# EspressoSystems/Push-CDN

Hardware: NVIDIA H100
Metric: broadcast fan-out egress GB/s (1 KiB x 2^20 subscribers per GPU, 1 topic); msgs/s and % of HBM peak alongside (higher is better)
Workload: dtype u8

## Files before the change

push-cdn_b200/csrc/kernels.cu:

```cuda
#include "kernels.cuh"

#include <atomic>

#include "frame_parse_core.h"

namespace pcdn {

std::atomic<unsigned long long> g_kernel_launches{0};
#define PCDN_COUNT_LAUNCH (void)g_kernel_launches.fetch_add(1, std::memory_order_relaxed)

unsigned long long kernel_launches() { return g_kernel_launches.load(std::memory_order_relaxed); }
void count_kernel_launch() { PCDN_COUNT_LAUNCH; }

__device__ __forceinline__ uint32_t lane_id() { return threadIdx.x & 31; }

__device__ __forceinline__ uint32_t warp_incl_scan(uint32_t v) {
  const uint32_t lane = lane_id();
#pragma unroll
  for (int o = 1; o < 32; o <<= 1) {
    uint32_t n = __shfl_up_sync(0xffffffffu, v, o);
    if (lane >= (uint32_t)o) v += n;
  }
  return v;
}
// ... 354 lines not shown
  const uint32_t p4 = p3 + __popc(hi.x), p5 = p4 + __popc(hi.y), p6 = p5 + __popc(hi.z), p7 = p6 + __popc(hi.w);
  const uint32_t incl = warp_incl_scan(p7), ex = incl - p7;
  uint32_t last = 0;
  if (lane == 31) {
    w.cnt[(size_t)j * s.nblk + blk] = incl;
    __threadfence();
    last = atomicAdd(&w.done[j], 1u) == s.nblk - 1 ? 1u : 0u;
  }
  uint4* Bo = reinterpret_cast<uint4*>(w.B + (size_t)j * s.W + w0);
  Bo[0] = lo; Bo[1] = hi;
  uint4 pre;
  pre.x = ex | ((ex + p0) << 16); pre.y = (ex + p1) | ((ex + p2) << 16);
  pre.z = (ex + p3) | ((ex + p4) << 16); pre.w = (ex + p5) | ((ex + p6) << 16);
  *reinterpret_cast<uint4*>(w.wpre + (size_t)j * s.W + w0) = pre;
  if (__shfl_sync(0xffffffffu, last, 31)) {
    __threadfence();
    uint32_t carry = 0;
    for (uint32_t bb = 0; bb < s.nblk; bb += 32) {
      const uint32_t i = bb + lane;
      const uint32_t v = i < s.nblk ? __ldcg(w.cnt + (size_t)j * s.nblk + i) : 0;
      const uint32_t in = warp_incl_scan(v);
      if (i < s.nblk) w.base[(size_t)j * s.nblk + i] = carry + in - v;
      carry += __shfl_sync(0xffffffffu, in, 31);
    }
    if (lane == 0) { w.D[m] = carry; w.jidx[m] = j; w.done[j] = 0; }
  }
}
void launch_match(const DevState& s, const Work& w, const BatchIn& b, cudaStream_t st) {
  if (!b.n_bcast) return;
  dim3 grid((s.nblk + 7) / 8, b.n_bcast);
  PCDN_COUNT_LAUNCH, k_match<<<grid, 256, 0, st>>>(s, b, w);
}

__device__ __forceinline__ uint32_t frame_vec_bytes(uint32_t raw_len) { return (4u + raw_len + 15u) & ~15u; }
__device__ __forceinline__ uint32_t frame_units(uint32_t raw_len) { return (4u + raw_len + kUnit - 1u) / kUnit; }
__device__ __forceinline__ uint32_t rec_units(const DevState& s, uint32_t raw_len) {
  return s.shared_payload ? 1u : frame_units(raw_len);
}
__device__ __forceinline__ uint32_t tile_recipients(uint32_t frame_bytes, uint32_t tile_bytes) {
  const uint32_t chunk = min(frame_bytes, kChunkBytes);
  return max(32u, min(kTileRecipients, tile_bytes / chunk));
}

__device__ __forceinline__ void plan_classify(const DevState& s, const BatchIn& b, uint32_t m, uint32_t d, uint32_t* cls_out,
                                              uint32_t* tiles_out) {
  uint32_t cls = CLS_THIN, tiles = 0;
  if (d >= kFatMin) {
    const uint32_t len = b.raw_len[m];
    const bool dense = s.cm_enable && ((uint64_t)d << kCmDenseShift) >= s.N && b.kind[m] == 4;
    if (dense && frame_units(len) * kUnit <= kCmMaxBytes) {
      cls = CLS_CM;
    } else {
      cls = CLS_FAT;
      const uint32_t nch = (frame_vec_bytes(len) + kChunkBytes - 1) / kChunkBytes;
      const uint32_t tr = tile_recipients(frame_vec_bytes(len), s.fat_tile_bytes);
      tiles = nch * ((d + tr - 1) / tr);
    }
  }
  *cls_out = cls; *tiles_out = tiles;
}

__global__ void __launch_bounds__(256) k_plan_a(DevState s, BatchIn b, Work w, uint32_t nblk) {
  __shared__ uint32_t sm[9];
  const uint32_t m = blockIdx.x * 256 + threadIdx.x;
  const bool valid = m < b.n_msgs;
  const uint32_t d = valid ? w.D[m] : 0;
  uint32_t cls, tiles;
  plan_classify(s, b, m, d, &cls, &tiles);
  uint32_t tot;
  uint32_t e0 = block256_excl_scan(cls != CLS_THIN ? d : 0, &tot, sm);
  if (threadIdx.x == 0) w.scan_tmp[blockIdx.x] = tot;
  uint32_t e1 = block256_excl_scan(cls == CLS_THIN ? d : 0, &tot, sm);
  if (threadIdx.x == 0) w.scan_tmp[nblk + blockIdx.x] = tot;
  uint32_t e2 = block256_excl_scan(tiles, &tot, sm);
  if (threadIdx.x == 0) w.scan_tmp[2 * nblk + blockIdx.x] = tot;
  uint32_t e3 = block256_excl_scan(cls == CLS_CM ? 1u : 0u, &tot, sm);
  if (threadIdx.x == 0) w.scan_tmp[3 * nblk + blockIdx.x] = tot;
  if (valid) { w.eb_fat[m] = e0; w.eb_thin[m] = e1; w.tbase[m] = e2; w.cm_rank[m] = e3; w.cls[m] = (uint8_t)cls; }
  if (gridDim.x == 1) {
    if (valid && cls == CLS_CM) w.cm_list[e3] = m;
    if (threadIdx.x == 0) {
      const uint32_t t0 = w.scan_tmp[0], t1 = w.scan_tmp[1], t2 = w.scan_tmp[2], t3 = w.scan_tmp[3];
      w.stats->n_fat_entries = t0; w.stats->n_thin_entries = t1; w.stats->n_fat_tiles = t2; w.stats->tile_cursor = 0;
      w.stats->n_cm = t3; w.stats->cm_cursor = 0;
      if (t0 > w.cap_fat || t1 > w.cap_thin) w.stats->status = 1;
      const uint32_t n = b.n_msgs;
      w.eb_fat[n] = t0; w.eb_thin[n] = t1; w.tbase[n] = t2; w.cm_rank[n] = t3;
    }
  }
}
__global__ void __launch_bounds__(256) k_plan_b(Work w, uint32_t nblk) {
  __shared__ uint32_t sm[9];
  const uint32_t q = blockIdx.x;
  uint32_t* t = w.scan_tmp + (size_t)q * nblk;
  uint32_t carry = 0;
  for (uint32_t bb = 0; bb < nblk; bb += 256) {
    const uint32_t i = bb + threadIdx.x;
    const uint32_t v = i < nblk ? t[i] : 0;
    uint32_t tot, ex = block256_excl_scan(v, &tot, sm);
    if (i < nblk) t[i] = ex + carry;
    carry += tot;
  }
  if (threadIdx.x == 0) {
    if (q == 0) { w.stats->n_fat_entries = carry; if (carry > w.cap_fat) w.stats->status = 1; }
    if (q == 1) { w.stats->n_thin_entries = carry; if (carry > w.cap_thin) w.stats->status = 1; }
    if (q == 2) { w.stats->n_fat_tiles = carry; w.stats->tile_cursor = 0; }
    if (q == 3) { w.stats->n_cm = carry; w.stats->cm_cursor = 0; }
  }
}
__global__ void __launch_bounds__(256) k_plan_c(BatchIn b, Work w, uint32_t nblk) {
  const uint32_t m = blockIdx.x * 256 + threadIdx.x;
  if (m < b.n_msgs) {
    w.eb_fat[m] += w.scan_tmp[blockIdx.x];
    w.eb_thin[m] += w.scan_tmp[nblk + blockIdx.x];
    w.tbase[m] += w.scan_tmp[2 * nblk + blockIdx.x];
    const uint32_t r = w.cm_rank[m] + w.scan_tmp[3 * nblk + blockIdx.x];
    w.cm_rank[m] = r;
    if (w.cls[m] == CLS_CM) w.cm_list[r] = m;
  } else if (m == b.n_msgs) {
    w.eb_fat[m] = w.stats->n_fat_entries;
    w.eb_thin[m] = w.stats->n_thin_entries;
    w.tbase[m] = w.stats->n_fat_tiles;
    w.cm_rank[m] = w.stats->n_cm;
  }
}
void launch_plan(const DevState& s, const Work& w, const BatchIn& b, cudaStream_t st) {
  if (b.n_bcast == 0) return;
  const uint32_t nblk = (b.n_msgs + 255) / 256;
  PCDN_COUNT_LAUNCH, k_plan_a<<<nblk, 256, 0, st>>>(s, b, w, nblk);
  if (nblk == 1) return;
  PCDN_COUNT_LAUNCH, k_plan_b<<<4, 256, 0, st>>>(w, nblk);
  PCDN_COUNT_LAUNCH, k_plan_c<<<(b.n_msgs + 1 + 255) / 256, 256, 0, st>>>(b, w, nblk);
}

struct ConnCursor {
  uint32_t pt, us, bu;
  uint32_t s1_off, s1_units, s1_rec, s2_units, s2_rec;
  uint32_t ovf, in2;
  uint32_t bytes;
};
__device__ __forceinline__ uint32_t alloc_record(ConnCursor& k, uint32_t u, uint32_t R, uint32_t raw_len) {
  if (k.ovf) return kOffInvalid;
  const bool wrap = k.pt + u > R;
  const uint32_t pad = wrap ? R - k.pt : 0, at = wrap ? 0 : k.pt;
  if (u > R || k.us + pad + u > R) { k.ovf = 1; return kOffInvalid; }
  k.us += pad + u;
  k.bu += pad + u;
  if (wrap && k.s1_rec) k.in2 = 1;
  if (!k.in2) { if (!k.s1_rec) k.s1_off = at; k.s1_units += u; k.s1_rec++; }
  else { k.s2_units += u; k.s2_rec++; }
  k.pt = at + u;
  k.bytes += 4u + raw_len;
  return at;
}

__device__ __forceinline__ uint32_t pool_lookback(const Work& w, uint32_t vb, uint32_t ctot) {
  const uint32_t lane = lane_id();
  volatile unsigned long long* st = w.lb_state;
  const unsigned long long tag = (unsigned long long)w.stamp << 34;
  auto pack = [&](uint32_t flag, uint32_t v) { return tag | ((unsigned long long)flag << 32) | v; };
  unsigned long long prefix64 = 0;
  if (vb > 0) {
    if (lane == 0) st[vb] = pack(1u, ctot);
    int j = (int)vb - 1;
    for (;;) {
      const int idx = j - (int)lane;
      unsigned long long x = 0;
      if (idx >= 0) { do { x = st[idx]; } while ((x >> 34) != (tag >> 34)); }
      const uint32_t flag = idx >= 0 ? (uint32_t)(x >> 32) & 3u : 2u;
      const uint32_t val = idx >= 0 ? (uint32_t)x : 0u;
      const uint32_t pm = __ballot_sync(0xffffffffu, flag == 2u);
      const int first = pm ? __ffs(pm) - 1 : 32;
      const uint32_t v = (int)lane <= first ? val : 0u;
      const unsigned long long take = ((unsigned long long)__reduce_add_sync(0xffffffffu, v >> 16) << 16) + __reduce_add_sync(0xffffffffu, v & 0xFFFFu);
      prefix64 += take;
      if (pm) break;
      j -= 32;
    }
  }
  const uint32_t prefix = (uint32_t)(prefix64 > 0xFFFFFFFFull ? 0xFFFFFFFFull : prefix64);
  const unsigned long long incl = prefix64 + ctot;
  if (lane == 0) { __threadfence(); st[vb] = pack(2u, incl > 0xFFFFFFFFull ? 0xFFFFFFFFu : (uint32_t)incl); }
  return prefix;
}
__device__ __forceinline__ void pool_allocate(const DevState& s, const Work& w, unsigned long long total64) {
  PoolState* p = s.pool_state;
  BatchStats* bs = w.stats;
  if (w.pool_unblock) p->blocked = 0;
  if (total64 > s.pool_units) { bs->status = 3; return; }
  const uint32_t total = (uint32_t)total64;
// ... 220 lines not shown
__global__ void __cluster_dims__(8, 1, 1) __launch_bounds__(1024, 1)
k_ctrl_small(DevState s, BatchIn b, Work w, int zero_stats, BatchStats* publish, int offsets_only) {
  __shared__ uint32_t sm[33];
  __shared__ uint32_t gbase[5];
  const uint32_t tid = threadIdx.x, rank = blockIdx.x;
  if (zero_stats && rank == 0 && tid < sizeof(BatchStats) / 4) reinterpret_cast<uint32_t*>(w.stats)[tid] = 0;

  if (HAS_DIRECT && rank == 0 && !offsets_only) {
    __shared__ uint32_t skey_s[kSmallCtrlMsgs], sorted_s[kSmallCtrlMsgs];
    __syncthreads();
    for (uint32_t g0 = 0; g0 < b.n_msgs * 8; g0 += 1024) direct_lookup_body<false>(s, b, w, g0 + tid);
    __syncthreads();
    const uint32_t n = b.n_msgs;
    if (tid < n) { const uint32_t t = w.dconn[tid]; skey_s[tid] = t == kConnNone ? s.N : t; }
    __syncthreads();
    if (tid < n) {
      const uint32_t key = skey_s[tid];
      uint32_t r = 0;
      for (uint32_t o = 0; o < n; o++) r += (skey_s[o] < key || (skey_s[o] == key && o < tid)) ? 1u : 0u;
      sorted_s[r] = key;
      w.dlist[r] = tid;
    }
    __syncthreads();
    if (tid < n) {
      const uint32_t key = sorted_s[tid];
      if (tid == 0 || sorted_s[tid - 1] != key) { w.dstart[key] = tid; w.dstamp[key] = w.stamp; }
      if (tid + 1 == n || sorted_s[tid + 1] != key) w.dend[key] = tid + 1;
    }
  }

  if (!offsets_only) {
    const uint32_t q = tid >> 8, wl = tid & 255u, nitems = b.n_bcast * s.nblk;
    for (uint32_t i0 = rank * 4; i0 < nitems; i0 += 32) {
      const uint32_t it = i0 + q;
      const bool live = it < nitems;
      const uint32_t j = live ? it / s.nblk : 0, blk = live ? it % s.nblk : 0;
      const uint32_t wd = blk * kBlockWords + wl;
      const uint32_t word = live ? match_word(s, b, b.bcast_index[j], wd) : 0;
      uint32_t tot, ex = cta_excl_scan<32>(__popc(word), &tot, sm);
      if (wl == 0) gbase[q] = ex;
      if (tid == 0) gbase[4] = tot;
      __syncthreads();
      if (live) {
        w.B[(size_t)j * s.W + wd] = word;
        w.wpre[(size_t)j * s.W + wd] = (uint16_t)(ex - gbase[q]);
        if (wl == 0) w.cnt[(size_t)j * s.nblk + blk] = gbase[q + 1] - gbase[q];
      }
      __syncthreads();
    }
  }
  cluster_sync_all();

  if (rank == 0 && !offsets_only) {
    if (tid < b.n_bcast) {
      uint32_t carry = 0;
      for (uint32_t blk = 0; blk < s.nblk; blk++) {
        const uint32_t v = w.cnt[(size_t)tid * s.nblk + blk];
        w.base[(size_t)tid * s.nblk + blk] = carry;
        carry += v;
      }
      const uint32_t m = b.bcast_index[tid];
      w.D[m] = carry; w.jidx[m] = tid;
    }
    __syncthreads();
  }

  if (rank == 0 && !offsets_only) {
    const uint32_t m = tid;
    const bool valid = m < b.n_msgs;
    const uint32_t d = valid ? w.D[m] : 0;
    uint32_t cls, tiles;
    plan_classify(s, b, m, d, &cls, &tiles);
    uint32_t t0, t1, t2, t3;
    const uint32_t e0 = cta_excl_scan<32>(cls != CLS_THIN ? d : 0, &t0, sm);
    const uint32_t e1 = cta_excl_scan<32>(cls == CLS_THIN ? d : 0, &t1, sm);
    const uint32_t e2 = cta_excl_scan<32>(tiles, &t2, sm);
    const uint32_t e3 = cta_excl_scan<32>(cls == CLS_CM ? 1u : 0u, &t3, sm);
    if (valid) {
      w.eb_fat[m] = e0; w.eb_thin[m] = e1; w.tbase[m] = e2; w.cm_rank[m] = e3; w.cls[m] = (uint8_t)cls;
      if (cls == CLS_CM) w.cm_list[e3] = m;
    }
    if (tid == 0) {
      w.stats->n_fat_entries = t0; w.stats->n_thin_entries = t1; w.stats->n_fat_tiles = t2; w.stats->tile_cursor = 0;
      w.stats->n_cm = t3; w.stats->cm_cursor = 0;
      if (t0 > w.cap_fat || t1 > w.cap_thin) w.stats->status = 1;
      const uint32_t n = b.n_msgs;
      w.eb_fat[n] = t0; w.eb_thin[n] = t1; w.tbase[n] = t2; w.cm_rank[n] = t3;
    }
  }
  cluster_sync_all();

  for (uint32_t c0 = 0; c0 < s.N; c0 += 8192)
    offsets_body<HAS_DIRECT, 1024, true, true>(s, b, w, s.N, c0 + rank * 1024 + tid, c0 / 1024 + rank, s.N / 1024);

  if (publish) {
    cluster_sync_all();
    if (rank == 0 && tid < sizeof(BatchStats) / 4)
      reinterpret_cast<uint32_t*>(publish)[tid] = __ldcg(reinterpret_cast<const uint32_t*>(w.stats) + tid);
  }
}
void launch_ctrl_small(const DevState& s, const Work& w, const BatchIn& b, bool has_direct, bool zero_stats,
                       BatchStats* publish, bool offsets_only, cudaStream_t st) {
  if (has_direct) PCDN_COUNT_LAUNCH, k_ctrl_small<true><<<8, 1024, 0, st>>>(s, b, w, zero_stats ? 1 : 0, publish, offsets_only ? 1 : 0);
  else PCDN_COUNT_LAUNCH, k_ctrl_small<false><<<8, 1024, 0, st>>>(s, b, w, zero_stats ? 1 : 0, publish, offsets_only ? 1 : 0);
}

__global__ void k_pool_retry_begin(BatchStats* bs) {
  bs->status = 0;
  bs->n_deliveries = 0; bs->bytes_out = 0;
  bs->n_spans = 0; bs->n_runs = 0; bs->n_overflow = 0;
  bs->tile_cursor = 0; bs->cm_cursor = 0;
}
void launch_pool_retry_begin(const DevState& s, const Work& w, cudaStream_t st) {
  cudaMemsetAsync(w.lb_state, 0, ((size_t)s.N / 256 + 1) * 8, st);
  PCDN_COUNT_LAUNCH, k_pool_retry_begin<<<1, 1, 0, st>>>(w.stats);
}

__device__ __forceinline__ uint8_t* conn_out(const DevState& s, const Work& w, uint32_t conn, uint32_t pool_base) {
  return s.pool ? s.rings + ((size_t)pool_base + w.cbase[conn]) * kUnit : s.rings + (size_t)conn * s.ring_bytes;
}

template <int VARIANT>
__device__ __forceinline__ void pack_fat_phase(const DevState& s, const BatchIn& b, const Work& w, uint8_t* buf,
                                               uint64_t* barp) {
  uint64_t& bar = *barp;
  __shared__ uint32_t t_info[8];
  const uint32_t tid = threadIdx.x, lane = tid & 31, warp = tid >> 5;
  const uint32_t ntiles = w.stats->n_fat_tiles;
  if (ntiles == 0) return;
  const uint32_t pool_base = w.stats->pool_base;
  uint32_t phase = 0;
  uint32_t staged_m = 0xFFFFFFFFu, staged_k = 0xFFFFFFFFu;

  uint32_t grab_next = 0, grab_left = 0;
  for (;;) {
    if (tid == 0) {
      if (grab_left == 0) { grab_next = atomicAdd(&w.stats->tile_cursor, s.fat_grab); grab_left = s.fat_grab; }
      const uint32_t t = grab_next++;
      grab_left--;
      t_info[0] = t;
      if (t < ntiles) {
        uint32_t lo = 0, hi = b.n_msgs;
        while (hi - lo > 1) { uint32_t mid = (lo + hi) >> 1; if (w.tbase[mid] <= t) lo = mid; else hi = mid; }
        const uint32_t m = lo, ltile = t - w.tbase[m], d = w.D[m];
        const uint32_t fb = frame_vec_bytes(b.raw_len[m]);
        const uint32_t tr = tile_recipients(fb, s.fat_tile_bytes);
        const uint32_t ngrp = (d + tr - 1) / tr;
        const uint32_t ch = ltile / ngrp, grp = ltile % ngrp;
        const uint32_t nbytes = min(kChunkBytes, fb - ch * kChunkBytes);
        t_info[1] = m; t_info[2] = ch; t_info[3] = grp * tr;
        t_info[4] = min(d, (grp + 1) * tr); t_info[5] = nbytes;
        t_info[6] = (m != staged_m || ch != staged_k) ? 1u : 0u;
        staged_m = m; staged_k = ch;
      }
    }
    __syncthreads();
    if (t_info[0] >= ntiles) break;
    const uint32_t m = t_info[1], ch = t_info[2], r0 = t_info[3], r1 = t_info[4], nbytes = t_info[5];
    if (t_info[6]) {
      if (VARIANT == 1) bulk_wait_read0();
      __syncthreads();
      if (tid == 0) {
        mbar_arrive_expect_tx(&bar, nbytes);
        bulk_g2s(buf, b.arena + (size_t)b.slot_off16[m] * 16 + (size_t)ch * kChunkBytes, nbytes, &bar);
      }
      mbar_wait(&bar, phase);
      phase ^= 1;
      if (ch == 0) {
        if (tid == 0) {
          *reinterpret_cast<uint32_t*>(buf) = bswap32(b.raw_len[m]);
          if (VARIANT == 1) fence_proxy_async_smem();
        }
        __syncthreads();
      }
    }
    const uint2* E = w.efat + w.eb_fat[m];
    const size_t chunk_off = (size_t)ch * kChunkBytes;
    const uint32_t nvec = nbytes >> 4;

    if (VARIANT == 1) {
      for (uint32_t r = r0 + tid; r < r1; r += 256) {
        const uint2 ent = E[r];
        if (ent.y != kOffInvalid)
          bulk_s2g(conn_out(s, w, ent.x, pool_base) + (size_t)ent.y * kUnit + chunk_off, buf, nbytes);
      }
      bulk_commit();
    } else if (nvec <= 128) {
      uint4 v0, v1, v2, v3;
      const uint4* sb = reinterpret_cast<const uint4*>(buf);
      v0 = lane < nvec ? sb[lane] : make_uint4(0, 0, 0, 0);
      v1 = lane + 32 < nvec ? sb[lane + 32] : make_uint4(0, 0, 0, 0);
      v2 = lane + 64 < nvec ? sb[lane + 64] : make_uint4(0, 0, 0, 0);
      v3 = lane + 96 < nvec ? sb[lane + 96] : make_uint4(0, 0, 0, 0);
      for (uint32_t r = r0 + warp * 32; r < r1; r += 8 * 32) {
        const uint2 ent = (r + lane < r1) ? E[r + lane] : make_uint2(0, kOffInvalid);
        const uint32_t cnt = min(32u, r1 - r);
        for (uint32_t i = 0; i < cnt; i++) {
          const uint32_t conn = __shfl_sync(0xffffffffu, ent.x, i), off = __shfl_sync(0xffffffffu, ent.y, i);
          if (off == kOffInvalid) continue;
          uint4* dst = reinterpret_cast<uint4*>(conn_out(s, w, conn, pool_base) + (size_t)off * kUnit + chunk_off);
          if (lane < nvec) st_stream16(dst + lane, v0);
          if (lane + 32 < nvec) st_stream16(dst + lane + 32, v1);
          if (lane + 64 < nvec) st_stream16(dst + lane + 64, v2);
          if (lane + 96 < nvec) st_stream16(dst + lane + 96, v3);
        }
      }
    } else {
      const uint4* sb = reinterpret_cast<const uint4*>(buf);
      for (uint32_t r = r0 + warp * 32; r < r1; r += 8 * 32) {
        const uint2 ent = (r + lane < r1) ? E[r + lane] : make_uint2(0, kOffInvalid);
        const uint32_t cnt = min(32u, r1 - r);
        for (uint32_t i = 0; i < cnt; i++) {
          const uint32_t conn = __shfl_sync(0xffffffffu, ent.x, i), off = __shfl_sync(0xffffffffu, ent.y, i);
          if (off == kOffInvalid) continue;
          uint4* dst = reinterpret_cast<uint4*>(conn_out(s, w, conn, pool_base) + (size_t)off * kUnit + chunk_off);
          for (uint32_t v = lane; v < nvec; v += 32) st_stream16(dst + v, sb[v]);
        }
      }
    }
    __syncthreads();
  }
  if (VARIANT == 1) bulk_wait_read0();
}

template <int VARIANT>
__device__ __forceinline__ void pack_cm_phase(const DevState& s, const BatchIn& b, const Work& w, uint8_t* buf,
                                              uint64_t* barp) {
  uint64_t& bar = *barp;
  __shared__ uint32_t g_m[kCmGroup], g_j[kCmGroup], g_soff[kCmGroup], g_units[kCmGroup], g_eb[kCmGroup];
  __shared__ uint32_t t_info[4];
  const uint32_t tid = threadIdx.x, lane = tid & 31, warp = tid >> 5;
  if (w.stats->status) return;
  const uint32_t ncm = w.stats->n_cm;
  if (ncm == 0) return;
  const uint32_t pool_base = w.stats->pool_base;
  const uint32_t ngroups = (ncm + kCmGroup - 1) / kCmGroup;
  const uint32_t tpg = s.W / kCmTileWords;
  const uint32_t ntiles = ngroups * tpg;
  uint32_t phase = 0;
  uint32_t staged_g = 0xFFFFFFFFu;

  for (;;) {
    if (tid == 0) {
      const uint32_t t = atomicAdd(&w.stats->cm_cursor, 1u);
      t_info[0] = t;
      if (t < ntiles) {
        const uint32_t g = t / tpg;
        const uint32_t gcount = min(kCmGroup, ncm - g * kCmGroup);
        t_info[1] = g; t_info[2] = gcount;
        t_info[3] = g != staged_g ? 1u : 0u;
        staged_g = g;
      }
    }
    __syncthreads();
    if (t_info[0] >= ntiles) break;
    const uint32_t gcount = t_info[2];
    if (t_info[3]) {
      if (VARIANT == 1) bulk_wait_read0();
      __syncthreads();
      if (tid == 0) {
        const uint32_t g = t_info[1];
        uint32_t soff = 0, total = 0;
        for (uint32_t i = 0; i < gcount; i++) {
          const uint32_t m = w.cm_list[g * kCmGroup + i];
          const uint32_t len = b.raw_len[m];
          g_m[i] = m; g_j[i] = w.jidx[m]; g_soff[i] = soff; g_units[i] = frame_units(len); g_eb[i] = w.eb_fat[m];
          soff += frame_units(len) * kUnit;
          total += frame_vec_bytes(len);
        }
        mbar_arrive_expect_tx(&bar, total);
        for (uint32_t i = 0; i < gcount; i++)
          bulk_g2s(buf + g_soff[i], b.arena + (size_t)b.slot_off16[g_m[i]] * 16, frame_vec_bytes(b.raw_len[g_m[i]]), &bar);
      }
      __syncthreads();
      mbar_wait(&bar, phase);
      phase ^= 1;
      if (tid < gcount) {
        *reinterpret_cast<uint32_t*>(buf + g_soff[tid]) = bswap32(b.raw_len[g_m[tid]]);
        if (VARIANT == 1) fence_proxy_async_smem();
      }
      __syncthreads();
    }
    const uint32_t wt = t_info[0] % tpg;
    for (uint32_t wi = warp; wi < kCmTileWords; wi += 8) {
      const uint32_t wd = wt * kCmTileWords + wi;
      const uint32_t myword = lane < gcount ? w.B[(size_t)g_j[lane] * s.W + wd] : 0u;
      const uint32_t any = __reduce_or_sync(0xffffffffu, myword);
      if (!any) continue;
      uint32_t offs[kCmGroup];
#pragma unroll
      for (int i = 0; i < (int)kCmGroup; i++) {
        const uint32_t wordi = __shfl_sync(0xffffffffu, myword, i);
        offs[i] = kOffInvalid;
        if ((uint32_t)i < gcount && ((wordi >> lane) & 1u)) {
          const uint32_t j = g_j[i];
          const uint32_t idx = g_eb[i] + w.base[(size_t)j * s.nblk + wd / kBlockWords] + w.wpre[(size_t)j * s.W + wd] +
                               __popc(wordi & ((1u << lane) - 1u));
          offs[i] = w.ecm[idx];
        }
      }
      if (VARIANT == 1) {
        uint8_t* ring = conn_out(s, w, wd * 32 + lane, pool_base);
        uint32_t run_o = kOffInvalid, run_units = 0, run_s = 0;
#pragma unroll
        for (int i = 0; i < (int)kCmGroup; i++) {
          const uint32_t o = offs[i];
          if (o != kOffInvalid && run_o != kOffInvalid && o == run_o + run_units) {
            run_units += g_units[i];
          } else {
            if (run_o != kOffInvalid) bulk_s2g(ring + (size_t)run_o * kUnit, buf + run_s, run_units * kUnit);
            run_o = o; run_s = g_soff[i]; run_units = (o != kOffInvalid) ? g_units[i] : 0;
          }
        }
        if (run_o != kOffInvalid) bulk_s2g(ring + (size_t)run_o * kUnit, buf + run_s, run_units * kUnit);
      } else {
        uint32_t rem = any;
        while (rem) {
          const int l = __ffs(rem) - 1;
          rem &= rem - 1;
          uint8_t* ring = conn_out(s, w, wd * 32 + l, pool_base);
          uint32_t run_o = kOffInvalid, run_units = 0, run_s = 0;
#pragma unroll
          for (int i = 0; i <= (int)kCmGroup; i++) {
            const uint32_t o = i < (int)kCmGroup ? __shfl_sync(0xffffffffu, offs[i < (int)kCmGroup ? i : 0], l) : kOffInvalid;
            if (o != kOffInvalid && run_o != kOffInvalid && o == run_o + run_units) {
              run_units += g_units[i];
            } else {
              if (run_o != kOffInvalid) {
                const uint4* src = reinterpret_cast<const uint4*>(buf + run_s);
                uint4* dst = reinterpret_cast<uint4*>(ring + (size_t)run_o * kUnit);
                const uint32_t nvec = run_units * 2;
                for (uint32_t v = lane; v < nvec; v += 128) {
                  const bool p1 = v + 32 < nvec, p2 = v + 64 < nvec, p3 = v + 96 < nvec;
                  uint4 x0 = src[v], x1, x2, x3;
                  if (p1) x1 = src[v + 32];
                  if (p2) x2 = src[v + 64];
                  if (p3) x3 = src[v + 96];
                  st_stream16(dst + v, x0);
                  if (p1) st_stream16(dst + v + 32, x1);
                  if (p2) st_stream16(dst + v + 64, x2);
                  if (p3) st_stream16(dst + v + 96, x3);
                }
              }
              run_o = o;
              if (i < (int)kCmGroup) { run_s = g_soff[i]; run_units = (o != kOffInvalid) ? g_units[i] : 0; }
            }
          }
        }
      }
    }
    if (VARIANT == 1) bulk_commit();
    __syncthreads();
  }
  if (VARIANT == 1) bulk_wait_read0();
}

__device__ __forceinline__ void copy_record(const uint4* __restrict__ src, uint4* __restrict__ dst, uint32_t raw_len, uint32_t lane) {
  const uint32_t nvec = (4u + raw_len + 15u) >> 4;
  const uint32_t hdr = bswap32(raw_len);
  for (uint32_t v = lane; v < nvec; v += 128) {
    uint4 x0, x1, x2, x3;
    const bool p1 = v + 32 < nvec, p2 = v + 64 < nvec, p3 = v + 96 < nvec;
    x0 = ld_nc16(src + v);
    if (p1) x1 = ld_nc16(src + v + 32);
    if (p2) x2 = ld_nc16(src + v + 64);
    if (p3) x3 = ld_nc16(src + v + 96);
    if (v == 0) x0.x = hdr;
    st_stream16(dst + v, x0);
    if (p1) st_stream16(dst + v + 32, x1);
    if (p2) st_stream16(dst + v + 64, x2);
    if (p3) st_stream16(dst + v + 96, x3);
  }
}
__device__ __forceinline__ void pack_thin_phase(const DevState& s, const BatchIn& b, const Work& w) {
  const uint32_t n = w.stats->n_thin_entries;
  const uint32_t pool_base = w.stats->pool_base;
  const uint32_t lane = lane_id();
  const uint32_t gw = (blockIdx.x * blockDim.x + threadIdx.x) >> 5, nw = (gridDim.x * blockDim.x) >> 5;
  for (uint32_t e = gw; e < n; e += nw) {
    const uint4 ent = w.ethin[e];
    if (ent.y == kOffInvalid) continue;
    copy_record(reinterpret_cast<const uint4*>(b.arena + (size_t)ent.z * 16),
                reinterpret_cast<uint4*>(conn_out(s, w, ent.x, pool_base) + (size_t)ent.y * kUnit), ent.w, lane);
  }
}
__device__ __forceinline__ void pack_direct_phase(const DevState& s, const BatchIn& b, const Work& w) {
  const uint32_t n = b.n_msgs;
  const uint32_t pool_base = w.stats->pool_base;
  const uint32_t lane = lane_id();
  const uint32_t gw = (blockIdx.x * blockDim.x + threadIdx.x) >> 5, nw = (gridDim.x * blockDim.x) >> 5;
  uint2 ent = make_uint2(0, kOffInvalid);
  uint32_t so = 0, len = 0;
  if (gw < n) { ent = w.edir[gw]; so = b.slot_off16[gw]; len = b.raw_len[gw]; }
  for (uint32_t m = gw; m < n; m += nw) {
    const uint2 cur = ent;
    const uint32_t cso = so, clen = len;
    const uint32_t nx = m + nw;
    if (nx < n) { ent = w.edir[nx]; so = b.slot_off16[nx]; len = b.raw_len[nx]; }
    if (cur.y == kOffInvalid) continue;
    copy_record(reinterpret_cast<const uint4*>(b.arena + (size_t)cso * 16),
                reinterpret_cast<uint4*>(conn_out(s, w, cur.x, pool_base) + (size_t)cur.y * kUnit), clen, lane);
  }
}

template <int VARIANT>
__global__ void __launch_bounds__(256) k_pack(DevState s, BatchIn b, Work w, int do_direct) {
  __shared__ __align__(128) uint8_t buf[kCmGroup * kCmMaxBytes];
  __shared__ __align__(8) uint64_t bars[2];
  if (w.stats->status) return;
  if (threadIdx.x == 0) {
    mbar_init(&bars[0], 1);
    mbar_init(&bars[1], 1);
    asm volatile("fence.mbarrier_init.release.cluster;" ::: "memory");
  }
  __syncthreads();
  pack_cm_phase<VARIANT>(s, b, w, buf, &bars[0]);
  __syncthreads();
  pack_fat_phase<VARIANT>(s, b, w, buf, &bars[1]);
  pack_thin_phase(s, b, w);
  if (do_direct) pack_direct_phase(s, b, w);
}
__global__ void __launch_bounds__(256, 8) k_pack_direct(DevState s, BatchIn b, Work w) {
  if (w.stats->status) return;
  pack_direct_phase(s, b, w);
}

__device__ __forceinline__ void st_ref_record(uint8_t* dst, uint32_t raw_len, uint32_t slot_off16, unsigned long long batch_id) {
  const unsigned long long off = (unsigned long long)slot_off16 * 16u + 4u;
  st_stream16(dst, make_uint4(0xFFFFFFFFu, bswap32(raw_len), (uint32_t)off, (uint32_t)(off >> 32)));
  st_stream16(dst + 16, make_uint4((uint32_t)batch_id, (uint32_t)(batch_id >> 32), 0u, 0u));
}
__global__ void __launch_bounds__(256) k_pack_ref(DevState s, BatchIn b, Work w, int do_direct) {
  if (w.stats->status) return;
  const uint32_t nfat = w.stats->n_fat_entries, nthin = w.stats->n_thin_entries;
  const uint64_t nft = (uint64_t)nfat + nthin, total = nft + (do_direct ? b.n_msgs : 0u);
  const uint32_t pool_base = w.stats->pool_base;
  const unsigned long long bid = w.batch_id;
  const uint64_t stride = (uint64_t)gridDim.x * blockDim.x;
  for (uint64_t i = (uint64_t)blockIdx.x * blockDim.x + threadIdx.x; i < total; i += stride) {
    uint32_t conn, off, m = 0, slot = 0, len = 0;
    bool thin = false;
    if (i < nfat) {
      const uint32_t e = (uint32_t)i;
      uint32_t lo = 0, hi = b.n_msgs;
      while (hi - lo > 1) { const uint32_t mid = (lo + hi) >> 1; if (w.eb_fat[mid] <= e) lo = mid; else hi = mid; }
      const uint2 ent = w.efat[e];
      conn = ent.x; off = ent.y; m = lo;
    } else if (i < nft) {
      const uint4 ent = w.ethin[i - nfat];
      conn = ent.x; off = ent.y; slot = ent.z; len = ent.w; thin = true;
    } else {
      m = (uint32_t)(i - nft);
      const uint2 ent = w.edir[m];
      conn = ent.x; off = ent.y;
    }
    if (off == kOffInvalid) continue;
    if (!thin) { slot = b.slot_off16[m]; len = b.raw_len[m]; }
    st_ref_record(conn_out(s, w, conn, pool_base) + (size_t)off * kUnit, len, slot, bid);
  }
}

void launch_pack(const DevState& s, const Work& w, const BatchIn& b, uint32_t n_direct, uint32_t variant, int n_sms, cudaStream_t st) {
  if (s.shared_payload) {
    if (b.n_bcast || n_direct) PCDN_COUNT_LAUNCH, k_pack_ref<<<(uint32_t)n_sms * 8, 256, 0, st>>>(s, b, w, n_direct ? 1 : 0);
    return;
  }
  const bool direct_separate = n_direct >= kThinSeparateMin;
  const uint32_t ctas_per_sm = ((variant >> 8) & 15u) ? ((variant >> 8) & 15u) : 3;
  const uint32_t grid = (uint32_t)n_sms * ctas_per_sm;
  const int do_direct = (n_direct && !direct_separate) ? 1 : 0;
  if (b.n_bcast || do_direct) {
    if (variant & 4) PCDN_COUNT_LAUNCH, k_pack<0><<<grid, 256, 0, st>>>(s, b, w, do_direct);
    else PCDN_COUNT_LAUNCH, k_pack<1><<<grid, 256, 0, st>>>(s, b, w, do_direct);
  }
  const uint32_t dctas = ((variant >> 12) & 15u) ? ((variant >> 12) & 15u) : 8u;
  if (direct_separate) PCDN_COUNT_LAUNCH, k_pack_direct<<<(uint32_t)n_sms * dctas, 256, 0, st>>>(s, b, w);
}

__global__ void __launch_bounds__(256) k_release(DevState s, const uint32_t* __restrict__ batch_units,
                                                 const BatchStats* __restrict__ stats) {
  if (stats->status) return;
  const uint32_t i = blockIdx.x * blockDim.x + threadIdx.x;
  if (i * 4 < s.N) {
    const uint4 u = reinterpret_cast<const uint4*>(batch_units)[i];
    if (u.x | u.y | u.z | u.w) {
      uint4* p = reinterpret_cast<uint4*>(s.used) + i;
      uint4 v = *p;
      v.x -= u.x; v.y -= u.y; v.z -= u.z; v.w -= u.w;
      *p = v;
// ... 20 lines not shown
```

push-cdn_b200/csrc/kernels.cuh:

```cuda
#pragma once
#include <cuda_runtime.h>
#include <stdint.h>

#include "hash.h"

namespace pcdn {

constexpr uint32_t kUnit = 32;
constexpr uint32_t kOffInvalid = 0xFFFFFFFFu;
constexpr uint32_t kConnNone = 0xFFFFFFFFu;
constexpr uint32_t kFatMin = 32;
constexpr uint32_t kChunkBytes = 16384;
constexpr uint32_t kTileRecipients = 1024;
constexpr uint32_t kBlockWords = 256;
constexpr uint32_t kCmGroup = 8;
constexpr uint32_t kCmMaxBytes = 4096;
constexpr uint32_t kSmallCtrlConns = 65536;
constexpr uint32_t kSmallCtrlMsgs = 256;
constexpr uint32_t kSmallCtrlItems = 256;
constexpr uint32_t kThinSeparateMin = 2048;
constexpr uint32_t kHotMin = 32;
constexpr uint32_t kHotCtas = 32;
constexpr uint32_t kCmTileWords = 16;
constexpr uint32_t kCmDenseShift = 4;
enum : uint8_t { CLS_THIN = 0, CLS_FAT = 1, CLS_CM = 2 };
enum : uint8_t {
  MSGF_USERS_ONLY = 1,
  MSGF_DEVPARSE = 2,
  MSGF_TOPICS_U8 = 4,
  MSGF_PRUNE = 8
};
constexpr int8_t kErrParse = -7, kErrPrune = -8;

struct DevState {
  uint32_t* sub;
  uint32_t* brk;
  uint32_t* owner_conn;
  CuckooEntry* cuckoo;
  uint8_t* keys;
  uint32_t* ptail;
  uint32_t* used;
  uint8_t* rings;
  uint32_t N, W, T, nblk;
  uint32_t bucket_mask, key_stride;
  uint32_t ring_units;
  uint32_t fat_tile_bytes;
  uint32_t fat_grab;
  uint32_t cm_enable;
  uint32_t n_valid_topics;
  uint32_t max_key_len;
  uint32_t pool;
  uint32_t pool_units;
  struct PoolState* pool_state;
  uint32_t conn_base;
  uint32_t span_runs;
  uint32_t count_drops;
  uint32_t shared_payload;
  uint64_t ring_bytes;
  uint64_t seed;
};

struct BatchIn {
  uint32_t n_msgs, n_bcast;
  const uint8_t* arena;
  const uint8_t* kind;
  const uint8_t* flags;
  const uint32_t* slot_off16;
  const uint32_t* raw_len;
  const uint32_t* aux_off;
  const uint32_t* aux_len;
  const uint16_t* topics;
  const uint32_t* bcast_index;
};

struct BatchStats {
  unsigned long long n_deliveries;
  unsigned long long bytes_out;
  uint32_t n_spans;
  uint32_t n_overflow;
  uint32_t n_direct_dropped;
  uint32_t status;
  uint32_t n_fat_entries;
  uint32_t n_thin_entries;
  uint32_t n_fat_tiles;
  uint32_t tile_cursor;
  uint32_t n_cm;
  uint32_t cm_cursor;
  uint32_t n_hot;
  uint32_t n_runs;
  uint32_t pool_base;
  uint32_t pool_units;
  uint32_t pool_skip;
  uint32_t reserved;
};

struct PoolState { uint32_t head, tail, used, blocked; };

struct Span { uint32_t conn, ring_off, len, n_records; };
struct SpanRun { uint32_t conn0, n_conns, ring_off, len, n_records, off_stride; };

struct Work {
  uint32_t* B;
  uint16_t* wpre;
  uint32_t* cnt;
  uint32_t* base;
  uint32_t* done;
  uint32_t* D;
  uint32_t* dconn;
  uint32_t* eb_fat;
  uint32_t* eb_thin;
  uint32_t* tbase;
  uint32_t* scan_tmp;
  uint8_t* cls;
  uint32_t* cm_rank;
  uint32_t* cm_list;
  uint32_t* jidx;
  uint2* efat;
  uint32_t* ecm;
  uint4* ethin;
  uint32_t cap_fat, cap_thin;
  uint32_t* dcount;
  uint32_t* dloc;
  uint32_t* dtile;
  uint32_t* dlist;
  uint32_t* hot_list;
  uint32_t* hot_bitmap;
  uint32_t* scan_done;
  uint2* edir;
  uint32_t* dstart;
  uint32_t* dend;
  uint32_t* dstamp;
  uint32_t stamp;
  uint32_t* cbase;
  unsigned long long* lb_state;
  uint32_t* lb_tot;
  uint32_t pool_unblock;
  unsigned long long batch_id;
  uint32_t* batch_units;
  Span* spans;
  uint32_t* overflow;
  int8_t* msg_status;
  BatchStats* stats;
};

struct Upd32 { uint32_t arr, idx, val; };
struct UpdSlot { uint32_t slot; CuckooEntry e; };

void launch_apply_updates(const DevState& s, const Upd32* u32, uint32_t n32, const UpdSlot* us,
                          uint32_t nslot, const uint32_t* key_slots, const uint8_t* key_bytes,
                          uint32_t nkeys, cudaStream_t st);
void launch_batch_begin(const DevState& s, const Work& w, const BatchIn& b, bool has_direct, cudaStream_t st);
void launch_parse(const DevState& s, const Work& w, const BatchIn& b, cudaStream_t st);
void launch_direct(const DevState& s, const Work& w, const BatchIn& b, uint32_t n_direct, cudaStream_t st);
void launch_match(const DevState& s, const Work& w, const BatchIn& b, cudaStream_t st);
void launch_plan(const DevState& s, const Work& w, const BatchIn& b, cudaStream_t st);
void launch_offsets(const DevState& s, const Work& w, const BatchIn& b, bool has_direct, int n_sms, cudaStream_t st);
void launch_ctrl_small(const DevState& s, const Work& w, const BatchIn& b, bool has_direct, bool zero_stats,
                       BatchStats* publish, bool offsets_only, cudaStream_t st);
void launch_pool_retry_begin(const DevState& s, const Work& w, cudaStream_t st);
void launch_pack(const DevState& s, const Work& w, const BatchIn& b, uint32_t n_direct, uint32_t variant, int n_sms, cudaStream_t st);
void launch_release(const DevState& s, const uint32_t* batch_units, const BatchStats* stats, cudaStream_t st);
void launch_pool_init(const DevState& s, cudaStream_t st);
unsigned long long kernel_launches();
void count_kernel_launch();

}
```

Before: 2928.

## Partition CM pack by static per-warp word ranges instead of atomic tile cursor

The CM pack phase drops the global atomic tile cursor (cm_cursor). Each warp now takes a fixed contiguous slice of subscriber words and loops over all message groups, staging each group once per CTA. Each warp precomputes the per-message rank for its lane and defers full-group contiguous bulk copies so they are issued together. kCmTileWords is halved and k_pack gets a minBlocks launch bound for occupancy. This risks load imbalance and register pressure in exchange for removing atomic contention and per-tile block syncs.

Measured after the change: 3036 (median of 6 runs). 3.7% higher.

```diff
diff --git a/push-cdn_b200/csrc/kernels.cu b/push-cdn_b200/csrc/kernels.cu
--- a/push-cdn_b200/csrc/kernels.cu
+++ b/push-cdn_b200/csrc/kernels.cu
@@ -460,7 +460,7 @@
     if (threadIdx.x == 0) {
       const uint32_t t0 = w.scan_tmp[0], t1 = w.scan_tmp[1], t2 = w.scan_tmp[2], t3 = w.scan_tmp[3];
       w.stats->n_fat_entries = t0; w.stats->n_thin_entries = t1; w.stats->n_fat_tiles = t2; w.stats->tile_cursor = 0;
-      w.stats->n_cm = t3; w.stats->cm_cursor = 0;
+      w.stats->n_cm = t3;
       if (t0 > w.cap_fat || t1 > w.cap_thin) w.stats->status = 1;
       const uint32_t n = b.n_msgs;
       w.eb_fat[n] = t0; w.eb_thin[n] = t1; w.tbase[n] = t2; w.cm_rank[n] = t3;
@@ -483,7 +483,7 @@
     if (q == 0) { w.stats->n_fat_entries = carry; if (carry > w.cap_fat) w.stats->status = 1; }
     if (q == 1) { w.stats->n_thin_entries = carry; if (carry > w.cap_thin) w.stats->status = 1; }
     if (q == 2) { w.stats->n_fat_tiles = carry; w.stats->tile_cursor = 0; }
-    if (q == 3) { w.stats->n_cm = carry; w.stats->cm_cursor = 0; }
+    if (q == 3) w.stats->n_cm = carry;
   }
 }
 __global__ void __launch_bounds__(256) k_plan_c(BatchIn b, Work w, uint32_t nblk) {
@@ -870,7 +870,7 @@
     }
     if (tid == 0) {
       w.stats->n_fat_entries = t0; w.stats->n_thin_entries = t1; w.stats->n_fat_tiles = t2; w.stats->tile_cursor = 0;
-      w.stats->n_cm = t3; w.stats->cm_cursor = 0;
+      w.stats->n_cm = t3;
       if (t0 > w.cap_fat || t1 > w.cap_thin) w.stats->status = 1;
       const uint32_t n = b.n_msgs;
       w.eb_fat[n] = t0; w.eb_thin[n] = t1; w.tbase[n] = t2; w.cm_rank[n] = t3;
@@ -897,7 +897,7 @@
   bs->status = 0;
   bs->n_deliveries = 0; bs->bytes_out = 0;
   bs->n_spans = 0; bs->n_runs = 0; bs->n_overflow = 0;
-  bs->tile_cursor = 0; bs->cm_cursor = 0;
+  bs->tile_cursor = 0;
 }
 void launch_pool_retry_begin(const DevState& s, const Work& w, cudaStream_t st) {
   cudaMemsetAsync(w.lb_state, 0, ((size_t)s.N / 256 + 1) * 8, st);
@@ -1016,129 +1016,128 @@
                                               uint64_t* barp) {
   uint64_t& bar = *barp;
   __shared__ uint32_t g_m[kCmGroup], g_j[kCmGroup], g_soff[kCmGroup], g_units[kCmGroup], g_eb[kCmGroup];
-  __shared__ uint32_t t_info[4];
   const uint32_t tid = threadIdx.x, lane = tid & 31, warp = tid >> 5;
   if (w.stats->status) return;
   const uint32_t ncm = w.stats->n_cm;
   if (ncm == 0) return;
   const uint32_t pool_base = w.stats->pool_base;
   const uint32_t ngroups = (ncm + kCmGroup - 1) / kCmGroup;
-  const uint32_t tpg = s.W / kCmTileWords;
-  const uint32_t ntiles = ngroups * tpg;
+  const uint32_t nwarps = gridDim.x * 8, gw = blockIdx.x * 8 + warp;
+  const uint32_t w_lo = (uint32_t)((uint64_t)gw * s.W / nwarps), w_hi = (uint32_t)((uint64_t)(gw + 1) * s.W / nwarps);
   uint32_t phase = 0;
-  uint32_t staged_g = 0xFFFFFFFFu;
-
-  for (;;) {
+
+  for (uint32_t g = 0; g < ngroups; g++) {
+    if (VARIANT == 1) bulk_wait_read0();
+    __syncthreads();
+    const uint32_t gcount = min(kCmGroup, ncm - g * kCmGroup);
     if (tid == 0) {
-      const uint32_t t = atomicAdd(&w.stats->cm_cursor, 1u);
-      t_info[0] = t;
-      if (t < ntiles) {
-        const uint32_t g = t / tpg;
-        const uint32_t gcount = min(kCmGroup, ncm - g * kCmGroup);
-        t_info[1] = g; t_info[2] = gcount;
-        t_info[3] = g != staged_g ? 1u : 0u;
-        staged_g = g;
-      }
-    }
-    __syncthreads();
-    if (t_info[0] >= ntiles) break;
-    const uint32_t gcount = t_info[2];
-    if (t_info[3]) {
-      if (VARIANT == 1) bulk_wait_read0();
-      __syncthreads();
-      if (tid == 0) {
-        const uint32_t g = t_info[1];
-        uint32_t soff = 0, total = 0;
-        for (uint32_t i = 0; i < gcount; i++) {
-          const uint32_t m = w.cm_list[g * kCmGroup + i];
-          const uint32_t len = b.raw_len[m];
-          g_m[i] = m; g_j[i] = w.jidx[m]; g_soff[i] = soff; g_units[i] = frame_units(len); g_eb[i] = w.eb_fat[m];
-          soff += frame_units(len) * kUnit;
-          total += frame_vec_bytes(len);
+      uint32_t soff = 0, total = 0;
+      for (uint32_t i = 0; i < gcount; i++) {
+        const uint32_t m = w.cm_list[g * kCmGroup + i];
+        const uint32_t len = b.raw_len[m];
+        g_m[i] = m; g_j[i] = w.jidx[m]; g_soff[i] = soff; g_units[i] = frame_units(len); g_eb[i] = w.eb_fat[m];
+        soff += frame_units(len) * kUnit;
+        total += frame_vec_bytes(len);
+      }
+      mbar_arrive_expect_tx(&bar, total);
+      for (uint32_t i = 0; i < gcount; i++)
+        bulk_g2s(buf + g_soff[i], b.arena + (size_t)b.slot_off16[g_m[i]] * 16, frame_vec_bytes(b.raw_len[g_m[i]]), &bar);
+    }
+    __syncthreads();
+    mbar_wait(&bar, phase);
+    phase ^= 1;
+    if (tid < gcount) {
+      *reinterpret_cast<uint32_t*>(buf + g_soff[tid]) = bswap32(b.raw_len[g_m[tid]]);
+      if (VARIANT == 1) fence_proxy_async_smem();
+    }
+    __syncthreads();
+    uint32_t group_units = 0;
+    for (uint32_t i = 0; i < gcount; i++) group_units += g_units[i];
+    const uint32_t jl = lane < gcount ? g_j[lane] : 0u, ebl = lane < gcount ? g_eb[lane] : 0u;
+
+    for (uint32_t wb = w_lo; wb < w_hi; wb += kCmTileWords) {
+      uint32_t run_at[kCmTileWords];
+#pragma unroll
+      for (uint32_t k = 0; k < kCmTileWords; k++) run_at[k] = kOffInvalid;
+#pragma unroll
+      for (uint32_t k = 0; k < kCmTileWords; k++) {
+        const uint32_t wd = wb + k;
+        if (wd >= w_hi) continue;
+        uint32_t myword = 0, myrank = 0;
+        if (lane < gcount) {
+          myword = w.B[(size_t)jl * s.W + wd];
+          myrank = ebl + w.base[(size_t)jl * s.nblk + wd / kBlockWords] + w.wpre[(size_t)jl * s.W + wd];
         }
-        mbar_arrive_expect_tx(&bar, total);
-        for (uint32_t i = 0; i < gcount; i++)
-          bulk_g2s(buf + g_soff[i], b.arena + (size_t)b.slot_off16[g_m[i]] * 16, frame_vec_bytes(b.raw_len[g_m[i]]), &bar);
-      }
-      __syncthreads();
-      mbar_wait(&bar, phase);
-      phase ^= 1;
-      if (tid < gcount) {
-        *reinterpret_cast<uint32_t*>(buf + g_soff[tid]) = bswap32(b.raw_len[g_m[tid]]);
-        if (VARIANT == 1) fence_proxy_async_smem();
-      }
-      __syncthreads();
-    }
-    const uint32_t wt = t_info[0] % tpg;
-    for (uint32_t wi = warp; wi < kCmTileWords; wi += 8) {
-      const uint32_t wd = wt * kCmTileWords + wi;
-      const uint32_t myword = lane < gcount ? w.B[(size_t)g_j[lane] * s.W + wd] : 0u;
-      const uint32_t any = __reduce_or_sync(0xffffffffu, myword);
-      if (!any) continue;
-      uint32_t offs[kCmGroup];
-#pragma unroll
-      for (int i = 0; i < (int)kCmGroup; i++) {
-        const uint32_t wordi = __shfl_sync(0xffffffffu, myword, i);
-        offs[i] = kOffInvalid;
-        if ((uint32_t)i < gcount && ((wordi >> lane) & 1u)) {
-          const uint32_t j = g_j[i];
-          const uint32_t idx = g_eb[i] + w.base[(size_t)j * s.nblk + wd / kBlockWords] + w.wpre[(size_t)j * s.W + wd] +
-                               __popc(wordi & ((1u << lane) - 1u));
-          offs[i] = w.ecm[idx];
-        }
-      }
-      if (VARIANT == 1) {
-        uint8_t* ring = conn_out(s, w, wd * 32 + lane, pool_base);
-        uint32_t run_o = kOffInvalid, run_units = 0, run_s = 0;
+        const uint32_t any = __reduce_or_sync(0xffffffffu, myword);
+        if (!any) continue;
+        uint32_t offs[kCmGroup];
 #pragma unroll
         for (int i = 0; i < (int)kCmGroup; i++) {
-          const uint32_t o = offs[i];
-          if (o != kOffInvalid && run_o != kOffInvalid && o == run_o + run_units) {
-            run_units += g_units[i];
-          } else {
-            if (run_o != kOffInvalid) bulk_s2g(ring + (size_t)run_o * kUnit, buf + run_s, run_units * kUnit);
-            run_o = o; run_s = g_soff[i]; run_units = (o != kOffInvalid) ? g_units[i] : 0;
-          }
+          const uint32_t wordi = __shfl_sync(0xffffffffu, myword, i), ranki = __shfl_sync(0xffffffffu, myrank, i);
+          offs[i] = kOffInvalid;
+          if ((uint32_t)i < gcount && ((wordi >> lane) & 1u)) offs[i] = w.ecm[ranki + __popc(wordi & ((1u << lane) - 1u))];
         }
-        if (run_o != kOffInvalid) bulk_s2g(ring + (size_t)run_o * kUnit, buf + run_s, run_units * kUnit);
-      } else {
-        uint32_t rem = any;
-        while (rem) {
-          const int l = __ffs(rem) - 1;
-          rem &= rem - 1;
-          uint8_t* ring = conn_out(s, w, wd * 32 + l, pool_base);
+        if (VARIANT == 1) {
+          uint8_t* ring = conn_out(s, w, wd * 32 + lane, pool_base);
           uint32_t run_o = kOffInvalid, run_units = 0, run_s = 0;
 #pragma unroll
-          for (int i = 0; i <= (int)kCmGroup; i++) {
-            const uint32_t o = i < (int)kCmGroup ? __shfl_sync(0xffffffffu, offs[i < (int)kCmGroup ? i : 0], l) : kOffInvalid;
+          for (int i = 0; i < (int)kCmGroup; i++) {
+            const uint32_t o = offs[i];
             if (o != kOffInvalid && run_o != kOffInvalid && o == run_o + run_units) {
               run_units += g_units[i];
             } else {
-              if (run_o != kOffInvalid) {
-                const uint4* src = reinterpret_cast<const uint4*>(buf + run_s);
-                uint4* dst = reinterpret_cast<uint4*>(ring + (size_t)run_o * kUnit);
-                const uint32_t nvec = run_units * 2;
-                for (uint32_t v = lane; v < nvec; v += 128) {
-                  const bool p1 = v + 32 < nvec, p2 = v + 64 < nvec, p3 = v + 96 < nvec;
-                  uint4 x0 = src[v], x1, x2, x3;
-                  if (p1) x1 = src[v + 32];
-                  if (p2) x2 = src[v + 64];
-                  if (p3) x3 = src[v + 96];
-                  st_stream16(dst + v, x0);
-                  if (p1) st_stream16(dst + v + 32, x1);
-                  if (p2) st_stream16(dst + v + 64, x2);
-                  if (p3) st_stream16(dst + v + 96, x3);
+              if (run_o != kOffInvalid) bulk_s2g(ring + (size_t)run_o * kUnit, buf + run_s, run_units * kUnit);
+              run_o = o; run_s = g_soff[i]; run_units = (o != kOffInvalid) ? g_units[i] : 0;
+            }
+          }
+          if (run_o != kOffInvalid) {
+            if (run_s == 0 && run_units == group_units) run_at[k] = run_o;
+            else bulk_s2g(ring + (size_t)run_o * kUnit, buf + run_s, run_units * kUnit);
+          }
+        } else {
+          uint32_t rem = any;
+          while (rem) {
+            const int l = __ffs(rem) - 1;
+            rem &= rem - 1;
+            uint8_t* ring = conn_out(s, w, wd * 32 + l, pool_base);
+            uint32_t run_o = kOffInvalid, run_units = 0, run_s = 0;
+#pragma unroll
+            for (int i = 0; i <= (int)kCmGroup; i++) {
+              const uint32_t o = i < (int)kCmGroup ? __shfl_sync(0xffffffffu, offs[i < (int)kCmGroup ? i : 0], l) : kOffInvalid;
+              if (o != kOffInvalid && run_o != kOffInvalid && o == run_o + run_units) {
+                run_units += g_units[i];
+              } else {
+                if (run_o != kOffInvalid) {
+                  const uint4* src = reinterpret_cast<const uint4*>(buf + run_s);
+                  uint4* dst = reinterpret_cast<uint4*>(ring + (size_t)run_o * kUnit);
+                  const uint32_t nvec = run_units * 2;
+                  for (uint32_t v = lane; v < nvec; v += 128) {
+                    const bool p1 = v + 32 < nvec, p2 = v + 64 < nvec, p3 = v + 96 < nvec;
+                    uint4 x0 = src[v], x1, x2, x3;
+                    if (p1) x1 = src[v + 32];
+                    if (p2) x2 = src[v + 64];
+                    if (p3) x3 = src[v + 96];
+                    st_stream16(dst + v, x0);
+                    if (p1) st_stream16(dst + v + 32, x1);
+                    if (p2) st_stream16(dst + v + 64, x2);
+                    if (p3) st_stream16(dst + v + 96, x3);
+                  }
                 }
+                run_o = o;
+                if (i < (int)kCmGroup) { run_s = g_soff[i]; run_units = (o != kOffInvalid) ? g_units[i] : 0; }
               }
-              run_o = o;
-              if (i < (int)kCmGroup) { run_s = g_soff[i]; run_units = (o != kOffInvalid) ? g_units[i] : 0; }
             }
           }
         }
       }
-    }
-    if (VARIANT == 1) bulk_commit();
-    __syncthreads();
+      if (VARIANT == 1) {
+#pragma unroll
+        for (uint32_t k = 0; k < kCmTileWords; k++)
+          if (run_at[k] != kOffInvalid)
+            bulk_s2g(conn_out(s, w, (wb + k) * 32 + lane, pool_base) + (size_t)run_at[k] * kUnit, buf, group_units * kUnit);
+        bulk_commit();
+      }
+    }
   }
   if (VARIANT == 1) bulk_wait_read0();
 }
@@ -1192,7 +1191,7 @@
 }
 
 template <int VARIANT>
-__global__ void __launch_bounds__(256) k_pack(DevState s, BatchIn b, Work w, int do_direct) {
+__global__ void __launch_bounds__(256, VARIANT == 1 ? 5 : 4) k_pack(DevState s, BatchIn b, Work w, int do_direct) {
   __shared__ __align__(128) uint8_t buf[kCmGroup * kCmMaxBytes];
   __shared__ __align__(8) uint64_t bars[2];
   if (w.stats->status) return;
diff --git a/push-cdn_b200/csrc/kernels.cuh b/push-cdn_b200/csrc/kernels.cuh
--- a/push-cdn_b200/csrc/kernels.cuh
+++ b/push-cdn_b200/csrc/kernels.cuh
@@ -21,7 +21,7 @@
 constexpr uint32_t kThinSeparateMin = 2048;
 constexpr uint32_t kHotMin = 32;
 constexpr uint32_t kHotCtas = 32;
-constexpr uint32_t kCmTileWords = 16;
+constexpr uint32_t kCmTileWords = 8;
 constexpr uint32_t kCmDenseShift = 4;
 enum : uint8_t { CLS_THIN = 0, CLS_FAT = 1, CLS_CM = 2 };
 enum : uint8_t {
@@ -85,7 +85,6 @@
   uint32_t n_fat_tiles;
   uint32_t tile_cursor;
   uint32_t n_cm;
-  uint32_t cm_cursor;
   uint32_t n_hot;
   uint32_t n_runs;
   uint32_t pool_base;
```
